# FKGSOFTWARE/TERRA-GAN

Hardware: AMD Instinct MI355X
Metric: DSM tiles/sec train-step (G+D) at 256x256 bs=16 (higher is better)
Workload: dtype f32; 1 GPU; BASELINE configs[1]: 256x256 1-ch DSM tiles, batch 16 per GPU, fp32, PConv-UNet G + PatchGAN D + L1/VGG-perceptual/TV/boundary(0.5) losses + 2x Adam; global_batch=16, tile=256, parallelism=single-gpu, launch=eager, vgg_weights=deterministic stand-in (ImageNet weights not fetchable offline; same FLOPs), vgg_trunk=forward Winograd F(2x2,3x3), dgrads F(4x4,3x3) (DESIGN 2b)

## Files before the change

terra-gan_amd/csrc/igemm_params.h:

```cpp
#pragma once
#include "common.h"

struct BnIn {
    const float *mean, *rstd, *gamma, *beta;
    int act;
    float slope;
};
struct IGemmParams {
    const float* src;
    const float* amask;
    const float* wmat;
    const float* bias;
    const float* rowscale;
    float* dst;
    float* ws;
    int B, IH, IW, C;
    int OH, OW, N, M;
    int DH, DW, ds, dy0, dx0;
    int TH, TW, ss, tstep, sy0, sx0;
    int KW, kstep, ky0, kx0;
    int Kfull, Ktot;
    int nchunks, T;
    int splits, steps_per_split;
    int act;
    float slope;
    int accumulate;
    int bf16;
    const float* gate;
    int gate_act;
    float gate_slope;
    const float* w_raw;
    long w_sn, w_sk, w_stap;
    float* wino_u;
    int wino4;
    int wino_ready;
    float* pool_dst;
    int pool_done;
    unsigned char* pool_code;
    int pool_only;
    BnIn in_bn;
    const uint32_t* gate_bits;
    int gate_bits_done;
    const TgSparseMap* sparse;
    int sparse_pix_done;
};
__device__ __forceinline__ float gate_factor(const IGemmParams& p, size_t idx) {
    const float gv = p.gate[idx];
    return gv > 0.f ? 1.f : (p.gate_act == TG_ACT_LEAKY ? p.gate_slope : 0.f);
}

int gate_bits_apply_launch(float* dx, const uint32_t* bits, int64_t rows, int C, hipStream_t s);

struct IGemmMulti {
    IGemmParams c[4];
    int zbeg[5];
};

struct WgradParams {
    const float* x;
    const float* amask;
    const float* dy;
    float* out;
    int B, H, W, C, Ho, Wo, Cout, k, stride, pad;
    int Mpix, Ktot, T, splits, steps_per_split;
    int nx, ny;
    int rowseg;
    BnIn in_bn;
};

enum SmallRoute {
    SR_NONE = 0,
    SR_C1MFMA = 100,
    SR_C1CONV = 110,
    SR_TO1CONVW = 200,
    SR_TO1_LDS = 300,
    SR_TO1_LDS_BNIN = 301,
    SR_TO1_LDS_MAP = 302,
    SR_TO1CONV64 = 400,
    SR_MULTI22_LDS = 500,
    SR_MULTI22 = 501,
    SR_C1WGRAD_MFMA = 600,
    SR_C1WGRAD_MFMA_BIAS = 610,
    SR_C1WGRAD = 620,
    SR_TO1WGRADW = 700,
    SR_TO1WGRAD_LDS = 800,
    SR_TO1WGRAD_LDS_BNIN = 801,
    SR_TO1WGRAD64 = 900,
};

enum WinoRoute {
    WR_NONE = 0,
    WR_FIRST = 1,
    WR_PIPE = WR_FIRST + 4,
    WR_QUEUED = WR_FIRST + 8,
    WR_MAP = WR_FIRST + 16,
    WR_MAP_LIST = WR_FIRST + 18,
    WR_W22_FAST = 2, WR_W22_QUEUED = 4,
    WR_WGRAD = WR_FIRST,
};

bool smallconv_fwd_applies(const IGemmParams& p);
int smallconv_fwd_launch(const IGemmParams& p, hipStream_t s, int* route = nullptr);
bool smallconv_to1_map_ok(const IGemmParams& p);
int pix_zero_launch(float* dx, const uint64_t* pix, int B, int H, int W, hipStream_t s);
bool smallconv_to1_multi_applies(const IGemmParams* cls, int ncls);
int smallconv_to1_multi_launch(const IGemmParams* cls, int ncls, hipStream_t s, int* route = nullptr);
bool smallconv_wgrad_applies(const WgradParams& p);
bool smallconv_bnin_fwd_ok(const IGemmParams& p);
bool smallconv_bnin_wgrad_ok(const WgradParams& p);
size_t smallconv_wgrad_ws_floats(const WgradParams& p);
int smallconv_wgrad_launch(const WgradParams& p, float* dw, float* ws, size_t ws_floats, hipStream_t s, float* db = nullptr,
                           int* db_done = nullptr, int* route = nullptr);
```

terra-gan_amd/csrc/wino22.inc:

```
#pragma once

struct W22Geom {
    int tiles_x, tiles_y, total_work, chunks_per_split, nt;
    int sy_min, sx_min;
    int s2d;
    int XH, XW, XC;
    int interleave;
    int* qctr;
    int ncls;
};
constexpr int W22_PTS = 9;
constexpr int W22_V = W22_PTS * 64 * 8;
constexpr int W22_PPIX = 17 * 17;
constexpr int W22_P = W22_PPIX * 8;
constexpr int W22_LDS_FLOATS = 4 * W22_V + W22_P + 8;

__device__ void wino22_weights_body(const float* __restrict__ w, float* __restrict__ U, int N, int K, const W22Weights& ww) {
    const int NT = N / WINO_BN;
    const size_t per = (size_t)N * K, total = per * ww.ncls;
    for (size_t idx0 = (size_t)blockIdx.x * 256 + threadIdx.x; idx0 < total; idx0 += (size_t)gridDim.x * 256) {
        const int cls = (int)(idx0 / per);
        const size_t idx = idx0 - cls * per;
        const int blk = (int)(idx >> 9), KC = K >> 3;
        const int k = (blk % KC) * 8 + (int)(idx & 7), n = (blk / KC) * WINO_BN + (int)((idx >> 3) & 63);
        const int ph = ww.by_phase ? k / ww.cin : cls, kc = ww.by_phase ? k - ph * ww.cin : k;
        const int dy = ph >> 1, dx = ph & 1;
        const float* wp = w + (size_t)n * ww.sn + (size_t)kc * ww.sk;
        float g[2][2];
#pragma unroll
        for (int u = 0; u < 2; ++u)
#pragma unroll
            for (int v = 0; v < 2; ++v) g[u][v] = wp[(size_t)((2 * ww.tyu[u] + dy) * 4 + (2 * ww.txv[v] + dx)) * ww.cin];
        const int row = n % WINO_BN;
        float* ub = U + cls * (per * W22_PTS) + ((size_t)(k >> 3) * NT + n / WINO_BN) * W22_V + row * 8 + wino_swz(row, k & 7);
        const float r0[3] = {g[0][0], g[0][0] + g[0][1], g[0][1]};
        const float r2[3] = {g[1][0], g[1][0] + g[1][1], g[1][1]};
#pragma unroll
        for (int b = 0; b < 3; ++b) {
            ub[(0 * 3 + b) * (WINO_BN * 8)] = r0[b];
            ub[(1 * 3 + b) * (WINO_BN * 8)] = r0[b] + r2[b];
            ub[(2 * 3 + b) * (WINO_BN * 8)] = r2[b];
        }
    }
}
__global__ __launch_bounds__(256) void wino22_weights_kernel(const float* __restrict__ w, float* __restrict__ U, int N, int K,
                                                             W22Weights ww) {
    wino22_weights_body(w, U, N, K, ww);
}

template <bool FAST, bool GATED, bool STEAL>
__global__ __launch_bounds__(WINO_THREADS) void wino22_kernel(const IGemmParams p, const W22Geom q, const float* __restrict__ U) {
    extern __shared__ __attribute__((aligned(16))) float smem[];
    float* Vs = smem;
    float* Us = smem + 2 * W22_V;
    float* Ps = smem + 4 * W22_V;

    const int tid = threadIdx.x, lane = tid & 63, wave = __builtin_amdgcn_readfirstlane(tid >> 6);
    const int mw = wave & 1, nw = (wave >> 1) & 1, xh = wave >> 2;
    __shared__ int wq_slot[2];
    WinoWork<STEAL> wk;
    wk.init(q.total_work, q.interleave, q.qctr, wq_slot);

    int n0, oy0, ox0, b, cls;
    const float* Ub;
    int s_iy[2], s_ix[2];
    int32_t poff[2];
    float pmul[2];
    int i_nt, i_tx, i_ty;
    auto locate = [&]() {
        const int item = wk.item;
        i_nt = item % q.nt;
        int tile = item / q.nt;
        cls = tile % q.ncls;
        tile /= q.ncls;
        i_tx = tile % q.tiles_x;
        tile /= q.tiles_x;
        i_ty = tile % q.tiles_y;
        b = tile / q.tiles_y;
    };
    const bool p1_ok = ((tid + WINO_THREADS) >> 1) < W22_PPIX;
    auto set_phase = [&](int ph) {
#pragma unroll
        for (int i = 0; i < 2; ++i) {
            int iy = s_iy[i], ix = s_ix[i], H = p.IH, W = p.IW, Cc = p.C;
            if (q.s2d) {
                iy = 2 * iy + (ph >> 1) - 1;
                ix = 2 * ix + (ph & 1) - 1;
                H = q.XH; W = q.XW; Cc = q.XC;
            }
            const bool ok = (i == 0 || p1_ok) && iy >= 0 && iy < H && ix >= 0 && ix < W;
            const int32_t pix = ok ? (b * H + iy) * W + ix : 0;
            poff[i] = pix * Cc + 4 * (tid & 1);
            if constexpr (FAST) poff[i] = ok ? poff[i] * 4 : (int32_t)0x80000000u;
            else pmul[i] = ok ? (p.amask ? p.amask[pix] : 1.f) : 0.f;
        }
    };
    const auto srsrc = __builtin_amdgcn_make_buffer_rsrc(
        const_cast<float*>(p.src), 0, FAST ? (int)(q.s2d ? (size_t)p.B * q.XH * q.XW * q.XC * 4 : (size_t)p.B * p.IH * p.IW * p.C * 4) : 0, 0x00020000);
    const auto ursrc = __builtin_amdgcn_make_buffer_rsrc(const_cast<float*>(U), 0, FAST ? (int)((size_t)q.ncls * W22_PTS * p.N * p.C * 4) : 0,
                                                         0x00020000);
    auto decode = [&]() {
        n0 = i_nt * WINO_BN; oy0 = i_ty * 16; ox0 = i_tx * 16;
        Ub = U + (size_t)cls * ((size_t)W22_PTS * p.N * p.C) + (size_t)i_nt * W22_V;
        const int py0 = oy0 + (q.ncls > 1 ? -(cls >> 1) : q.sy_min), px0 = ox0 + (q.ncls > 1 ? -(cls & 1) : q.sx_min);
#pragma unroll
        for (int i = 0; i < 2; ++i) {
            const int pp = (tid + WINO_THREADS * i) >> 1, spy = pp / 17, spx = pp - spy * 17;
            s_iy[i] = py0 + spy;
            s_ix[i] = px0 + spx;
        }
    };
    const int c_begin = blockIdx.z * q.chunks_per_split;
    const int c_end = min(p.C >> 3, c_begin + q.chunks_per_split);
    const int c_last = c_end - 1;
    const size_t ustep = (size_t)q.nt * W22_V;
    const int cpp = q.s2d ? (q.XC >> 3) : (p.C >> 3);
    const int ph_begin = c_begin / cpp;

    f32x4 ru[3], rp[2];
    int cur_ph, c_base, c_next;
    auto start_phase = [&](int ph) { cur_ph = ph; c_base = ph * cpp; c_next = c_base + cpp; set_phase(ph); };
    auto pload1 = [&](int c, int i) {
        if constexpr (FAST) rp[i] = __builtin_bit_cast(f32x4, __builtin_amdgcn_raw_buffer_load_b128(srsrc, poff[i], (c - c_base) * 32, 0));
        else rp[i] = *reinterpret_cast<const f32x4*>(p.src + poff[i] + (c - c_base) * 8);
    };
    const int u_idx[3] = {tid, tid + WINO_THREADS, tid < 128 ? tid + 2 * WINO_THREADS : tid};
    const size_t u_base = (size_t)W22_PTS * p.N * p.C;
    auto uload1 = [&](int c, int j) {
        if constexpr (FAST)
            ru[j] = __builtin_bit_cast(f32x4, __builtin_amdgcn_raw_buffer_load_b128(
                ursrc, 16 * u_idx[j], (int)(((size_t)cls * u_base + (size_t)i_nt * W22_V + (size_t)c * ustep) * 4), 0));
        else ru[j] = *reinterpret_cast<const f32x4*>(Ub + (size_t)c * ustep + 4 * u_idx[j]);
    };
    auto pstore1 = [&](int i) {
        f32x4 v = rp[i];
        if constexpr (!FAST) {
            v = v * pmul[i];
#pragma unroll
            for (int e = 0; e < 4; ++e) v[e] = pmul[i] != 0.f ? v[e] : 0.f;
        }
        if (i == 0 || p1_ok) *reinterpret_cast<f32x4*>(Ps + 4 * (tid + WINO_THREADS * i)) = v;
    };
    auto ustore1 = [&](int buf, int j) {
        if (j < 2 || tid < 128) *reinterpret_cast<f32x4*>(Us + buf * W22_V + 4 * (tid + WINO_THREADS * j)) = ru[j];
    };

    const int t_quad = lane & 1, t_tile = (lane >> 1) + 32 * (wave & 1), t_a = min(wave >> 1, 2);
    const bool t_on = wave < 6;
    const int t_src0 = ((2 * (t_tile >> 3) + t_a) * 17 + 2 * (t_tile & 7)) * 8 + 4 * t_quad;
    const int t_src1 = ((2 * (t_tile >> 3) + 1) * 17 + 2 * (t_tile & 7)) * 8 + 4 * t_quad;
    const int t_dst = (t_a * 3) * 512 + t_tile * 8 + (((t_quad ^ (t_tile >> 4)) & 1) << 2);
    f32x4 td[2][3], tt[3];
    auto t_read1 = [&](int k) {
        td[k / 3][k % 3] = *reinterpret_cast<const f32x4*>(Ps + ((k / 3) ? t_src1 : t_src0) + (k % 3) * 8);
    };
    auto t_row1 = [&](int j) {
        if (t_a == 1) tt[j] = td[0][j];
        else tt[j] = td[0][j] - td[1][j];
    };
    auto t_col1 = [&](int buf, int k) {
        const f32x4 v = k == 0 ? tt[0] - tt[1] : k == 1 ? tt[1] : tt[2] - tt[1];
        *reinterpret_cast<f32x4*>(Vs + buf * W22_V + t_dst + k * 512) = v;
    };

    const int pt0 = xh == 0 ? 0 : 6;
    const int arow = 32 * mw + (lane & 31), brow = 32 * nw + (lane & 31);
    const int a_off = pt0 * 512 + arow * 8 + ((((lane >> 5) ^ (arow >> 4)) & 1) << 2);
    const int b_off = pt0 * 512 + brow * 8 + ((((lane >> 5) ^ (brow >> 4)) & 1) << 2);

    if (wk.item < 0 || c_begin >= c_end) { wk.done(q.qctr); return; }
    locate();
    decode();
    start_phase(ph_begin);
#pragma unroll
    for (int i = 0; i < 2; ++i) pload1(c_begin, i);
#pragma unroll
    for (int j = 0; j < 3; ++j) uload1(c_begin, j);

    for (;;) {
        f32x16 acc[6];
#pragma unroll
        for (int i = 0; i < 6; ++i)
#pragma unroll
            for (int r = 0; r < 16; ++r) acc[i][r] = 0.f;
        {
#pragma unroll
            for (int i = 0; i < 2; ++i) pstore1(i);
#pragma unroll
            for (int j = 0; j < 3; ++j) ustore1(0, j);
            {
                const int c1 = min(c_begin + 1, c_last);
                if (c1 >= c_next) start_phase(cur_ph + 1);
#pragma unroll
                for (int i = 0; i < 2; ++i) pload1(c1, i);
#pragma unroll
                for (int j = 0; j < 3; ++j) uload1(c1, j);
            }
            wino_barrier();
            if (t_on) {
#pragma unroll
                for (int k = 0; k < 6; ++k) t_read1(k);
#pragma unroll
                for (int j = 0; j < 3; ++j) t_row1(j);
#pragma unroll
                for (int k = 0; k < 3; ++k) t_col1(0, k);
            }
            wino_barrier();
            f32x4 fa[2], fb[2];
            fa[0] = *reinterpret_cast<const f32x4*>(Vs + a_off);
            fb[0] = *reinterpret_cast<const f32x4*>(Us + b_off);
            int cur = 0;
            for (int c = c_begin; c < c_end; ++c) {
                const int nxt = cur ^ 1;
                const int c2 = min(c + 2, c_last);
                const float* Vc = Vs + cur * W22_V + a_off;
                const float* Uc = Us + cur * W22_V + b_off;
                const float* Vn = Vs + nxt * W22_V + a_off;
                const float* Un = Us + nxt * W22_V + b_off;
                wino_static_for(std::make_integer_sequence<int, 24>{}, [&](auto tc) {
                    constexpr int t = decltype(tc)::value;
                    constexpr int xi = t >> 2, e = t & 3;
                    if constexpr (t < 2) pstore1(t);
                    if constexpr (t == 2) {
                        if (c2 >= c_next) start_phase(cur_ph + 1);
                        pload1(c2, 0);
                    }
                    if constexpr (t == 3) pload1(c2, 1);
                    if constexpr (t == 4) wino_barrier();
                    if constexpr (t >= 5 && t < 8) { if (t_on) { t_read1(t - 5); t_read1(3 + t - 5); } }
                    if constexpr (t >= 8 && t < 11) { if (t_on) t_row1(t - 8); }
                    if constexpr (t >= 12 && t < 15) { if (t_on) t_col1(nxt, t - 12); }
                    if constexpr (t >= 15 && t < 18) ustore1(nxt, t - 15);
                    if constexpr (t >= 18 && t < 21) uload1(c2, t - 18);
                    if constexpr (t == 21) wino_barrier();
                    if constexpr (e == 0 && xi < 5) {
                        if (xi + 1 < 3 || xh == 0) {
                            fa[(xi + 1) & 1] = *reinterpret_cast<const f32x4*>(Vc + (xi + 1) * 512);
                            fb[(xi + 1) & 1] = *reinterpret_cast<const f32x4*>(Uc + (xi + 1) * 512);
                        }
                    }
                    if constexpr (t == 22) {
                        fa[0] = *reinterpret_cast<const f32x4*>(Vn);
                        fb[0] = *reinterpret_cast<const f32x4*>(Un);
                    }
                    __builtin_amdgcn_sched_barrier(0);
                    if (xi < 3 || xh == 0) acc[xi] = __builtin_amdgcn_mfma_f32_32x32x2f32(fa[xi & 1][e], fb[xi & 1][e], acc[xi], 0, 0, 0);
                    __builtin_amdgcn_sched_barrier(0);
                });
                cur = nxt;
            }
        }
        const int e_n0 = n0, e_oy0 = oy0, e_ox0 = ox0, e_b = b, e_cls = cls;
        const int wq_next = wk.next(wq_slot);
        const bool more_items = wq_next >= 0;
        const int wq_pulled = wk.request(wq_next);
        wino_barrier();

        float* X = smem;
        float* scratch = smem + 2 * W22_V + wave * (32 * 36);
        f32x16 own[2];
#pragma unroll
        for (int j = 0; j < 2; ++j) {
            float* xs = X + ((nw * 2 + mw) * 2 + j) * 1024 + lane;
            if (xh == 0) {
#pragma unroll
                for (int r = 0; r < 16; ++r) {
                    const float s0 = acc[j][r] + acc[j + 1][r], s1 = acc[3 + j][r] + acc[4 + j][r];
                    own[j][r] = s0 + s1;
                    xs[r * 64] = s1;
                }
            } else {
#pragma unroll
                for (int r = 0; r < 16; ++r) own[j][r] = acc[j][r] + acc[j + 1][r];
            }
        }
        if (more_items) {
            wk.item = wq_next;
            locate();
            decode();
            start_phase(ph_begin);
#pragma unroll
            for (int i = 0; i < 2; ++i) pload1(c_begin, i);
#pragma unroll
            for (int j = 0; j < 3; ++j) uload1(c_begin, j);
        }
        wino_barrier();
        const int e_dy0 = q.ncls > 1 ? 1 - (e_cls >> 1) : p.dy0, e_dx0 = q.ncls > 1 ? 1 - (e_cls & 1) : p.dx0;
        f32x4 bq = {0.f, 0.f, 0.f, 0.f};
        float rsq[2][4] = {{1.f, 1.f, 1.f, 1.f}, {1.f, 1.f, 1.f, 1.f}};
        if (p.splits == 1) {
            if (p.bias) bq = *reinterpret_cast<const f32x4*>(p.bias + e_n0 + 32 * nw + 4 * (lane & 7));
            if (p.rowscale) {
#pragma unroll
                for (int j = 0; j < 2; ++j)
#pragma unroll
                    for (int t4 = 0; t4 < 4; ++t4) {
                        const int t = 32 * mw + (lane >> 3) + 8 * t4;
                        const int oy = min(e_oy0 + 2 * (t >> 3) + xh, p.OH - 1), ox = min(e_ox0 + 2 * (t & 7) + j, p.OW - 1);
                        rsq[j][t4] = p.rowscale[((size_t)e_b * p.DH + (oy * p.ds + e_dy0)) * p.DW + (ox * p.ds + e_dx0)];
                    }
            }
        }
        f32x4 gq[GATED ? 2 : 1][GATED ? 4 : 1];
        if constexpr (GATED) {
#pragma unroll
            for (int j = 0; j < 2; ++j)
#pragma unroll
                for (int t4 = 0; t4 < 4; ++t4) {
                    const int t = 32 * mw + (lane >> 3) + 8 * t4;
                    const int oy = min(e_oy0 + 2 * (t >> 3) + xh, p.OH - 1), ox = min(e_ox0 + 2 * (t & 7) + j, p.OW - 1);
                    const size_t pix = ((size_t)e_b * p.DH + (oy * p.ds + e_dy0)) * p.DW + (ox * p.ds + e_dx0);
                    gq[j][t4] = *reinterpret_cast<const f32x4*>(p.gate + pix * p.N + e_n0 + 32 * nw + 4 * (lane & 7));
                }
        }
#pragma unroll
        for (int j = 0; j < 2; ++j) {
            f32x16 y = own[j];
            if (xh == 1) {
                const float* xr = X + ((nw * 2 + mw) * 2 + j) * 1024 + lane;
#pragma unroll
                for (int r = 0; r < 16; ++r) y[r] += xr[r * 64];
            }
            tile_rows4i(scratch, y, lane, [&](int t4, int rr, int cc, f32x4 v4) {
                const int t = 32 * mw + rr;
                const int oy = e_oy0 + 2 * (t >> 3) + xh, ox = e_ox0 + 2 * (t & 7) + j;
                const int nb = e_n0 + 32 * nw + cc;
                if (oy >= p.OH || ox >= p.OW) return;
                if (p.splits > 1) {
                    const size_t m = ((size_t)e_b * p.OH + oy) * p.OW + ox;
                    *reinterpret_cast<f32x4*>(p.ws + (((size_t)e_cls * p.splits + blockIdx.z) * p.M + m) * p.N + nb) = v4;
                } else {
                    const size_t pix = ((size_t)e_b * p.DH + (oy * p.ds + e_dy0)) * p.DW + (ox * p.ds + e_dx0);
                    *reinterpret_cast<f32x4*>(p.dst + pix * p.N + nb) = epilogue4(p, v4, pix, nb, GATED ? &gq[GATED ? j : 0][GATED ? t4 : 0] : nullptr, &rsq[j][t4], &bq);
                }
            });
        }
        wk.publish(wq_pulled, wq_slot);
        if (!more_items) break;
        wino_barrier();
        wk.advance(wq_next);
    }
    wk.done(q.qctr);
}

static bool wino22_enabled() {
    static const bool off = getenv("TG_NO_WINO") != nullptr || getenv("TG_NO_WINO22") != nullptr;
    return !off;
}
static bool wino22_fwd_geom_ok(const TgConv* g) {
    return wino22_enabled() && g->precision != TG_PREC_BF16 && g->k == 4 && g->stride == 2 && g->pad == 1 && (g->H % 2) == 0 &&
           (g->W % 2) == 0 && g->Ho == g->H / 2 && g->Wo == g->W / 2 && (g->Cin % 8) == 0 && (g->Cout % WINO_BN) == 0 && g->Ho >= 16 &&
           g->Wo >= 16;
}
static bool wino22_dgrad_geom_ok(const TgConv* g) {
    return wino22_enabled() && g->precision != TG_PREC_BF16 && g->k == 4 && g->stride == 2 && g->pad == 1 && (g->H % 2) == 0 &&
           (g->W % 2) == 0 && g->Ho == g->H / 2 && g->Wo == g->W / 2 && (g->Cout % 8) == 0 && (g->Cin % WINO_BN) == 0 && g->Ho >= 16 &&
           g->Wo >= 16;
}
static size_t wino22_u_floats(const TgConv* g) { return align_up((size_t)4 * W22_PTS * g->Cin * g->Cout, 64); }

static int launch_wino22(const TgConv* g, IGemmParams& p, int dgrad, size_t ws_floats_avail, hipStream_t s) {
    W22Geom q = {};
    W22Weights ww = {};
    p.B = g->B;
    p.OH = g->Ho; p.OW = g->Wo;
    p.M = g->B * g->Ho * g->Wo;
    ww.cin = g->Cin;
    if (!dgrad) {
        p.IH = g->Ho + 1; p.IW = g->Wo + 1; p.C = 4 * g->Cin; p.N = g->Cout;
        p.DH = g->Ho; p.DW = g->Wo; p.ds = 1; p.dy0 = 0; p.dx0 = 0;
        q.s2d = 1; q.XH = g->H; q.XW = g->W; q.XC = g->Cin; q.ncls = 1;
        q.sy_min = 0; q.sx_min = 0;
        ww.sn = 16L * g->Cin; ww.sk = 1; ww.by_phase = 1; ww.ncls = 1; ww.k_fast = 1;
        ww.tyu[0] = 0; ww.tyu[1] = 1; ww.txv[0] = 0; ww.txv[1] = 1;
    } else {
        p.IH = g->Ho; p.IW = g->Wo; p.C = g->Cout; p.N = g->Cin;
        p.DH = g->H; p.DW = g->W; p.ds = 2;
        q.s2d = 0; q.ncls = 4;
        ww.sn = 1; ww.sk = 16L * g->Cin; ww.by_phase = 0; ww.ncls = 4; ww.k_fast = 0;
        ww.tyu[0] = 1; ww.tyu[1] = 0; ww.txv[0] = 1; ww.txv[1] = 0;
    }
    q.tiles_x = cdiv(p.OW, 16);
    q.tiles_y = cdiv(p.OH, 16);
    q.nt = p.N / WINO_BN;
    q.total_work = q.tiles_x * q.tiles_y * p.B * q.nt * q.ncls;
    q.interleave = wino_interleave_ok((size_t)W22_PTS * p.N * p.C * sizeof(float));
    const int nchunks = p.C / 8;
    int splits = 1;
    if (nchunks >= 16) {
        int smax = nchunks / 8 < 16 ? nchunks / 8 : 16;
        while (smax > 1 && (size_t)smax * p.M * p.N * q.ncls > ws_floats_avail) --smax;
        splits = choose_splits(q.total_work, smax, WINO_PLAN_CUS);
    }
    q.chunks_per_split = cdiv(nchunks, splits);
    p.splits = cdiv(nchunks, q.chunks_per_split);
    p.Ktot = 4 * p.C;
    TgWprepItem it = {};
    it.kind = 3; it.N = p.N; it.K = p.C; it.w = p.w_raw; it.out = p.wino_u; it.w22 = ww;
    int rc = TG_OK;
    const auto transform = [&]() -> int {
        hipLaunchKernelGGL(wino22_weights_kernel, dim3(ew_grid((int64_t)p.N * p.C * q.ncls, 256)), dim3(256), 0, s, p.w_raw, p.wino_u, p.N,
                           p.C, ww);
        TG_CHECK_LAUNCH("wino22_weights_kernel");
        return TG_OK;
    };
    if (wino_prep(p, it, transform, &rc)) return rc;
    static const bool no_fast = getenv("TG_WINO_NO_FAST") != nullptr;
    const size_t src_bytes = (size_t)g->B * (dgrad ? (size_t)g->Ho * g->Wo * g->Cout : (size_t)g->H * g->W * g->Cin) * 4;
    const bool fast = !no_fast && p.amask == nullptr && src_bytes < ((size_t)1 << 31) && wino22_u_floats(g) * 4 < ((size_t)1 << 31);
    const bool gated = p.gate != nullptr && p.splits == 1;
    typedef void (*W22Kern)(const IGemmParams, const W22Geom, const float*);
    static const W22Kern kerns[8] = {wino22_kernel<false, false, false>, wino22_kernel<false, true, false>, wino22_kernel<true, false, false>,
                                     wino22_kernel<true, true, false>, wino22_kernel<false, false, true>, wino22_kernel<false, true, true>,
                                     wino22_kernel<true, false, true>, wino22_kernel<true, true, true>};
    static LdsOptIn opts[8];
    q.qctr = wino_queue_block(s, p.splits, q.total_work);
    const int ki = (q.qctr ? 4 : 0) + (fast ? 2 : 0) + (gated ? 1 : 0);
    const double mtot = (double)p.M * q.ncls;
    const WinoProf pf = {0, 4022, (int)mtot, 2.0 * mtot * (double)p.N * p.Ktot,
                         4.0 * ((double)g->B * (dgrad ? g->Ho * g->Wo * g->Cout : g->H * g->W * g->Cin) + 16.0 * g->Cin * g->Cout +
                                mtot * p.N + (p.rowscale ? mtot : 0.0)), WR_FIRST + ki};
    if ((rc = wino_launch(kerns[ki], opts[ki], (size_t)W22_LDS_FLOATS * sizeof(float), "wino22_kernel", p, q, pf, false, s))) return rc;
    if (p.splits > 1) {
        IGemmMulti pm = {};
        for (int c = 0; c < q.ncls; ++c) {
            pm.c[c] = p;
            pm.c[c].ws = p.ws + (size_t)c * p.splits * p.M * p.N;
            if (q.ncls > 1) { pm.c[c].dy0 = 1 - (c >> 1); pm.c[c].dx0 = 1 - (c & 1); }
        }
        hipLaunchKernelGGL(igemm_splitk_epilogue_multi, dim3(ew_grid((int64_t)p.M * p.N, 256), q.ncls), dim3(256), 0, s, pm);
        TG_CHECK_LAUNCH("igemm_splitk_epilogue_multi");
    }
    return TG_OK;
}

struct W22WgradGeom {
    int strips_x, tiles_y, nstrips, steps_per_split, splits, ntco, ntci, ctiles;
};
constexpr int W22_XR = 3 * 17 * WG_PITCH;
constexpr int W22_DR = 2 * 16 * WG_PITCH;
constexpr int W22_WG_LDS_FLOATS = 4 * W22_V + W22_XR + W22_DR;

__global__ __launch_bounds__(WINO_THREADS) void wino22_wgrad_kernel(const WgradParams p, const W22WgradGeom q, float* __restrict__ slabs) {
    extern __shared__ __attribute__((aligned(16))) float smem[];
    float* As = smem;
    float* Bs = smem + 2 * W22_V;
    float* Xr = smem + 4 * W22_V;
    float* Dr = Xr + W22_XR;

    const int tid = threadIdx.x, lane = tid & 63, wave = __builtin_amdgcn_readfirstlane(tid >> 6);
    const int mw = wave & 1, nw = (wave >> 1) & 1, xh = wave >> 2;
    const int work = xcd_remap(blockIdx.x, q.ntco * q.ntci * q.splits);
    const int tco = work % q.ntco, tci = (work / q.ntco) % q.ntci, split = work / (q.ntco * q.ntci);
    const int ph = tci / q.ctiles, ct = tci - ph * q.ctiles;
    const int pdy = (ph >> 1) - 1, pdx = (ph & 1) - 1;
    const int s_begin = split * q.steps_per_split;
    const int s_end = min(q.nstrips, s_begin + q.steps_per_split);

    const int k = lane & 7, qd = (lane >> 3) + 8 * (wave & 1), a = min(wave >> 1, 2);
    const bool t_on = wave < 6;
    int icol[4];
#pragma unroll
    for (int e = 0; e < 4; ++e) icol[e] = (3 * a) * 512 + (qd + 16 * e) * 8 + ((((k >> 2) ^ e) & 1) << 2) + (k & 3);
    const int xrd0 = (a * 17 + 2 * k) * WG_PITCH + 4 * qd, xrd1 = (17 + 2 * k) * WG_PITCH + 4 * qd;
    const int drd = (2 * k) * WG_PITCH + 4 * qd;

    const auto xrsrc = __builtin_amdgcn_make_buffer_rsrc(const_cast<float*>(p.x), 0, (int)((size_t)p.B * p.H * p.W * p.C * 4), 0x00020000);
    const auto drsrc = __builtin_amdgcn_make_buffer_rsrc(const_cast<float*>(p.dy), 0, (int)((size_t)p.B * p.Ho * p.Wo * p.Cout * 4), 0x00020000);
    const uint32_t OOB = 0xFFFFFFF0u;

    int xs_r[2], xs_px[2], xs_lds[2];
    bool xs_on[2];
#pragma unroll
    for (int i = 0; i < 2; ++i) {
        const int idx = tid + WINO_THREADS * i;
        const int ps = idx >> 4;
        xs_on[i] = ps < 3 * 17;
        xs_r[i] = ps / 17;
        xs_px[i] = ps - xs_r[i] * 17;
        xs_lds[i] = ps * WG_PITCH + 4 * (idx & 15);
    }
    const uint32_t xs_ch = (uint32_t)(ct * 64 + 4 * (tid & 15)) * 4u;
    const int ds_i = tid >> 8, ds_px = (tid >> 4) & 15, ds_lds = (tid >> 4) * WG_PITCH + 4 * (tid & 15);
    const uint32_t ds_ch = (uint32_t)(tco * 64 + 4 * (tid & 15)) * 4u;

    f32x4 rx[2][2], rd[2];
    int ls = s_begin, lsx = s_begin % q.strips_x, lty = (s_begin / q.strips_x) % q.tiles_y, lb = s_begin / (q.strips_x * q.tiles_y);
    auto raw_load = [&](auto setc) {
        constexpr int SET = decltype(setc)::value;
        const bool live = ls < s_end;
#pragma unroll
        for (int i = 0; i < 2; ++i) {
            const int py = 2 * (2 * lty + xs_r[i]) + pdy, px = 2 * (16 * lsx + xs_px[i]) + pdx;
            const bool ok = live && xs_on[i] && py >= 0 && py < p.H && px >= 0 && px < p.W;
            const uint32_t off = ok ? (((uint32_t)(lb * p.H + py) * p.W + px) * (uint32_t)p.C) * 4u + xs_ch : OOB;
            rx[SET][i] = __builtin_bit_cast(f32x4, __builtin_amdgcn_raw_buffer_load_b128(xrsrc, off, 0, 0));
        }
        {
            const int oy = 2 * lty + ds_i, ox = 16 * lsx + ds_px;
            const bool ok = live && oy < p.Ho && ox < p.Wo;
            const uint32_t off = ok ? (((uint32_t)(lb * p.Ho + oy) * p.Wo + ox) * (uint32_t)p.Cout) * 4u + ds_ch : OOB;
            rd[SET] = __builtin_bit_cast(f32x4, __builtin_amdgcn_raw_buffer_load_b128(drsrc, off, 0, 0));
        }
        ++ls;
        if (++lsx == q.strips_x) { lsx = 0; if (++lty == q.tiles_y) { lty = 0; ++lb; } }
    };
    auto raw_store = [&](auto setc) {
        constexpr int SET = decltype(setc)::value;
#pragma unroll
        for (int i = 0; i < 2; ++i)
            if (xs_on[i]) *reinterpret_cast<f32x4*>(Xr + xs_lds[i]) = rx[SET][i];
        *reinterpret_cast<f32x4*>(Dr + ds_lds) = rd[SET];
    };
    using Set0 = std::integral_constant<int, 0>;
    using Set1 = std::integral_constant<int, 1>;
    f32x4 xr[2][3], dr[2][2], tt[3], rr[2];
    auto x_read = [&](int j) {
        xr[0][j] = *reinterpret_cast<const f32x4*>(Xr + xrd0 + j * WG_PITCH);
        xr[1][j] = *reinterpret_cast<const f32x4*>(Xr + xrd1 + j * WG_PITCH);
    };
    auto d_read = [&](int i) {
        dr[i][0] = *reinterpret_cast<const f32x4*>(Dr + drd + (i * 16) * WG_PITCH);
        dr[i][1] = *reinterpret_cast<const f32x4*>(Dr + drd + (i * 16 + 1) * WG_PITCH);
    };
    auto x_rows = [&]() {
#pragma unroll
        for (int j = 0; j < 3; ++j) {
            if (a == 1) tt[j] = xr[0][j];
            else tt[j] = xr[0][j] - xr[1][j];
        }
    };
    auto d_rows = [&]() {
#pragma unroll
        for (int j = 0; j < 2; ++j) rr[j] = a == 0 ? dr[0][j] : (a == 1 ? dr[0][j] + dr[1][j] : dr[1][j]);
    };
    auto x_out = [&](int buf, int b, int h) {
        const f32x4 v = b == 0 ? tt[0] - tt[1] : b == 1 ? tt[1] : tt[2] - tt[1];
        float* dst = Bs + buf * W22_V + b * 512;
        dst[icol[2 * h]] = v[2 * h];
        dst[icol[2 * h + 1]] = v[2 * h + 1];
    };
    auto d_out = [&](int buf, int b, int h) {
        const f32x4 v = b == 0 ? rr[0] : b == 1 ? rr[0] + rr[1] : rr[1];
        float* dst = As + buf * W22_V + b * 512;
        dst[icol[2 * h]] = v[2 * h];
        dst[icol[2 * h + 1]] = v[2 * h + 1];
    };

    const int pt0 = xh == 0 ? 0 : 6;
    const int arow = 32 * mw + (lane & 31), brow = 32 * nw + (lane & 31);
    const int a_off = pt0 * 512 + arow * 8 + ((((lane >> 5) ^ (arow >> 4)) & 1) << 2);
    const int b_off = pt0 * 512 + brow * 8 + ((((lane >> 5) ^ (brow >> 4)) & 1) << 2);

    f32x16 acc[6];
#pragma unroll
    for (int i = 0; i < 6; ++i)
#pragma unroll
        for (int r = 0; r < 16; ++r) acc[i][r] = 0.f;

    if (s_begin < s_end) {
        raw_load(Set0{});
        raw_store(Set0{});
        raw_load(Set0{});
        raw_load(Set1{});
        wino_barrier();
        if (t_on) {
#pragma unroll
            for (int j = 0; j < 3; ++j) x_read(j);
            d_read(0);
            d_read(1);
            x_rows();
            d_rows();
#pragma unroll
            for (int b = 0; b < 3; ++b) { x_out(0, b, 0); x_out(0, b, 1); d_out(0, b, 0); d_out(0, b, 1); }
        }
        wino_barrier();
        f32x4 fa[2], fb[2];
        fa[0] = *reinterpret_cast<const f32x4*>(As + a_off);
        fb[0] = *reinterpret_cast<const f32x4*>(Bs + b_off);
        int cur = 0;
        auto kstep = [&](auto setc) {
            const int nxt = cur ^ 1;
            const float* Ac = As + cur * W22_V + a_off;
            const float* Bc = Bs + cur * W22_V + b_off;
            const float* An = As + nxt * W22_V + a_off;
            const float* Bn = Bs + nxt * W22_V + b_off;
            wino_static_for(std::make_integer_sequence<int, 24>{}, [&](auto tc) {
                constexpr int t = decltype(tc)::value;
                constexpr int xi = t >> 2, e = t & 3;
                if constexpr (t == 0) raw_store(setc);
                if constexpr (t == 1) raw_load(setc);
                if constexpr (t == 2) wino_barrier();
                if constexpr (t >= 3 && t < 6) { if (t_on) x_read(t - 3); }
                if constexpr (t == 6) { if (t_on) { d_read(0); d_read(1); } }
                if constexpr (t == 7) { if (t_on) x_rows(); }
                if constexpr (t >= 8 && t < 14) { if (t_on) x_out(nxt, (t - 8) >> 1, t & 1); }
                if constexpr (t == 13) { if (t_on) d_rows(); }
                if constexpr (t >= 14 && t < 20) { if (t_on) d_out(nxt, (t - 14) >> 1, t & 1); }
                if constexpr (t == 20) wino_barrier();
                if constexpr (e == 0 && xi < 5) {
                    if (xi + 1 < 3 || xh == 0) {
                        fa[(xi + 1) & 1] = *reinterpret_cast<const f32x4*>(Ac + (xi + 1) * 512);
                        fb[(xi + 1) & 1] = *reinterpret_cast<const f32x4*>(Bc + (xi + 1) * 512);
                    }
                }
                if constexpr (t == 22) {
                    fa[0] = *reinterpret_cast<const f32x4*>(An);
                    fb[0] = *reinterpret_cast<const f32x4*>(Bn);
                }
                __builtin_amdgcn_sched_barrier(0);
                if (xi < 3 || xh == 0) acc[xi] = __builtin_amdgcn_mfma_f32_32x32x2f32(fa[xi & 1][e], fb[xi & 1][e], acc[xi], 0, 0, 0);
                __builtin_amdgcn_sched_barrier(0);
            });
            cur = nxt;
        };
        for (int s = s_begin; s < s_end; s += 2) {
            kstep(Set0{});
            if (s + 1 < s_end) kstep(Set1{});
        }
    }
    float* slab = slabs + ((size_t)work * W22_PTS + pt0) * 4096;
    const int npts = xh == 0 ? 6 : 3;
#pragma unroll
    for (int i = 0; i < 6; ++i) {
        if (i < npts) {
#pragma unroll
            for (int r = 0; r < 16; ++r) {
                const int row = 32 * mw + (r & 3) + 8 * (r >> 2) + 4 * (lane >> 5);
                slab[(size_t)i * 4096 + row * 64 + 32 * nw + (lane & 31)] = acc[i][r];
            }
        }
    }
}

__global__ __launch_bounds__(256) void wino22_wgrad_reduce_kernel(const float* __restrict__ slabs, float* __restrict__ dw, int Cout,
                                                                  int Cin, int ntco, int ntci, int splits) {
    const int total = Cout * 4 * Cin;
    const int ctiles = Cin / 64;
    for (int idx = blockIdx.x * 256 + threadIdx.x; idx < total; idx += gridDim.x * 256) {
        const int col = idx & 63, row = (idx >> 6) & 63, tile = idx >> 12;
        const int tco = tile % ntco, tci = tile / ntco;
        float u[W22_PTS];
#pragma unroll
        for (int i = 0; i < W22_PTS; ++i) u[i] = 0.f;
        const size_t sstride = (size_t)ntci * ntco * W22_PTS * 4096;
        const float* sl = slabs + ((size_t)tile * W22_PTS) * 4096 + row * 64 + col;
        int sp = 0;
        for (; sp + 4 <= splits; sp += 4) {
            float v[4][W22_PTS];
#pragma unroll
            for (int k = 0; k < 4; ++k)
#pragma unroll
                for (int i = 0; i < W22_PTS; ++i) v[k][i] = sl[(size_t)(sp + k) * sstride + (size_t)i * 4096];
#pragma unroll
            for (int k = 0; k < 4; ++k)
#pragma unroll
                for (int i = 0; i < W22_PTS; ++i) u[i] += v[k][i];
        }
        for (; sp < splits; ++sp)
#pragma unroll
            for (int i = 0; i < W22_PTS; ++i) u[i] += sl[(size_t)sp * sstride + (size_t)i * 4096];
        const int ph = tci / ctiles, ct = tci - ph * ctiles;
        const int co = tco * 64 + 4 * (row & 15) + (row >> 4), c = ct * 64 + 4 * (col & 15) + (col >> 4);
        const int dy = ph >> 1, dx = ph & 1;
#pragma unroll
        for (int ty = 0; ty < 2; ++ty)
#pragma unroll
            for (int tx = 0; tx < 2; ++tx)
                dw[((size_t)(co * 4 + 2 * ty + dy) * 4 + 2 * tx + dx) * Cin + c] =
                    (u[ty * 3 + tx] + u[ty * 3 + tx + 1]) + (u[(ty + 1) * 3 + tx] + u[(ty + 1) * 3 + tx + 1]);
    }
}

static bool wino22_wgrad_ok(const TgConv* g, const float* in_mask) {
    static const bool off = getenv("TG_NO_WINO22_WGRAD") != nullptr;
    if (off || !wino22_enabled() || in_mask != nullptr || g->precision == TG_PREC_BF16) return false;
    if (g->k != 4 || g->stride != 2 || g->pad != 1 || (g->H % 2) || (g->W % 2) || g->Ho != g->H / 2 || g->Wo != g->W / 2) return false;
    if ((g->Cin % 64) != 0 || (g->Cout % 64) != 0 || g->Ho < 16 || g->Wo < 16) return false;
    if ((size_t)g->B * g->H * g->W * g->Cin * 4 >= ((size_t)1 << 31) || (size_t)g->B * g->Ho * g->Wo * g->Cout * 4 >= ((size_t)1 << 31))
        return false;
    return true;
}
static W22WgradGeom wino22_wgrad_plan(const TgConv* g) {
    W22WgradGeom q = {};
    q.strips_x = cdiv(g->Wo, 16);
    q.tiles_y = cdiv(g->Ho, 2);
    q.nstrips = g->B * q.tiles_y * q.strips_x;
    q.ntco = g->Cout / 64;
    q.ctiles = g->Cin / 64;
    q.ntci = 4 * q.ctiles;
    const int tiles = q.ntco * q.ntci;
    int smax = q.nstrips / 8 < 512 ? q.nstrips / 8 : 512;
    if (smax < 1) smax = 1;
    const int splits = choose_splits_k(tiles, smax, WINO_PLAN_CUS, q.nstrips, 0.03);
    q.steps_per_split = cdiv(q.nstrips, splits);
    q.splits = cdiv(q.nstrips, q.steps_per_split);
    return q;
}
static size_t wino22_wgrad_ws_floats(const TgConv* g) {
    if (!wino22_wgrad_ok(g, nullptr)) return 0;
    const W22WgradGeom q = wino22_wgrad_plan(g);
    return (size_t)q.splits * q.ntco * q.ntci * W22_PTS * 4096;
}
static int launch_wino22_wgrad(const TgConv* g, const WgradParams& p, float* dw, float* ws, hipStream_t s) {
    const W22WgradGeom q = wino22_wgrad_plan(g);
    const size_t lds = (size_t)W22_WG_LDS_FLOATS * sizeof(float);
    static LdsOptIn opt;
    if (int rc = lds_opt_in(opt, reinterpret_cast<const void*>(wino22_wgrad_kernel), lds, "wino22 wgrad")) return rc;
    {
        const double by = 4.0 * ((double)p.B * p.H * p.W * p.C + (double)p.Mpix * p.Cout + (double)p.Cout * p.Ktot);
        ProfScope ps(s, 1, 2.0 * p.Mpix * (double)p.Cout * p.Ktot, by, p.Cout, p.Ktot, p.Mpix, p.C, q.splits, 4122);
        ps.r.route = WR_WGRAD;
        hipLaunchKernelGGL(wino22_wgrad_kernel, dim3(q.ntco * q.ntci * q.splits), dim3(WINO_THREADS), lds, s, p, q, ws);
    }
    TG_CHECK_LAUNCH("wino22_wgrad_kernel");
    hipLaunchKernelGGL(wino22_wgrad_reduce_kernel, dim3(ew_grid((int64_t)g->Cout * 4 * g->Cin, 256)), dim3(256), 0, s, ws, dw, g->Cout,
                       g->Cin, q.ntco, q.ntci, q.splits);
    TG_CHECK_LAUNCH("wino22_wgrad_reduce_kernel");
    return TG_OK;
}
```

Before: 1077 tiles/s.

## Add wide-N Winograd F(2x2) kernel computing two output-channel tiles per block

Adds a wino22w kernel in which each work item covers 2*WINO_BN output channels, so every input-tile transform is shared across twice as many filters and the work count is halved. It is enabled by default when the fast path applies, N divides evenly, there is no split-K, and enough work remains to fill the CUs. The aim is to cut redundant input loads and transforms per FLOP. In exchange it uses more LDS and registers per block, which can lower occupancy, and leaves fewer work items for load balancing.

```diff
diff --git a/terra-gan_amd/csrc/igemm_params.h b/terra-gan_amd/csrc/igemm_params.h
--- a/terra-gan_amd/csrc/igemm_params.h
+++ b/terra-gan_amd/csrc/igemm_params.h
@@ -96,6 +96,7 @@
     WR_MAP = WR_FIRST + 16,
     WR_MAP_LIST = WR_FIRST + 18,
     WR_W22_FAST = 2, WR_W22_QUEUED = 4,
+    WR_W22_WIDE = 8,
     WR_WGRAD = WR_FIRST,
 };
 
diff --git a/terra-gan_amd/csrc/wino22.inc b/terra-gan_amd/csrc/wino22.inc
--- a/terra-gan_amd/csrc/wino22.inc
+++ b/terra-gan_amd/csrc/wino22.inc
@@ -343,9 +343,267 @@
     wk.done(q.qctr);
 }
 
+constexpr int W22W_U = 2 * W22_V;
+constexpr int W22W_LDS_FLOATS = 2 * W22_V + 2 * W22W_U + W22_P + 8;
+
+template <bool GATED, bool STEAL>
+__global__ __launch_bounds__(WINO_THREADS) void wino22w_kernel(const IGemmParams p, const W22Geom q, const float* __restrict__ U) {
+    extern __shared__ __attribute__((aligned(16))) float smem[];
+    float* Vs = smem;
+    float* Us = smem + 2 * W22_V;
+    float* Ps = smem + 2 * W22_V + 2 * W22W_U;
+
+    const int tid = threadIdx.x, lane = tid & 63, wave = __builtin_amdgcn_readfirstlane(tid >> 6);
+    const int mw = wave & 1, nw = wave >> 1;
+    __shared__ int wq_slot[2];
+    WinoWork<STEAL> wk;
+    wk.init(q.total_work, q.interleave, q.qctr, wq_slot);
+
+    int n0, oy0, ox0, b, cls;
+    int py0, px0;
+    int32_t poff[2];
+    int i_nt, i_tx, i_ty;
+    auto locate = [&]() {
+        const int item = wk.item;
+        i_nt = item % q.nt;
+        int tile = item / q.nt;
+        cls = tile % q.ncls;
+        tile /= q.ncls;
+        i_tx = tile % q.tiles_x;
+        tile /= q.tiles_x;
+        i_ty = tile % q.tiles_y;
+        b = tile / q.tiles_y;
+    };
+    const bool p1_ok = ((tid + WINO_THREADS) >> 1) < W22_PPIX;
+    auto set_phase = [&](int ph) {
+        int st = tid;
+        asm volatile("" : "+v"(st));
+#pragma unroll
+        for (int i = 0; i < 2; ++i) {
+            const int pp = (st + WINO_THREADS * i) >> 1, spy = pp / 17, spx = pp - spy * 17;
+            int iy = py0 + spy, ix = px0 + spx, H = p.IH, W = p.IW, Cc = p.C;
+            if (q.s2d) {
+                iy = 2 * iy + (ph >> 1) - 1;
+                ix = 2 * ix + (ph & 1) - 1;
+                H = q.XH; W = q.XW; Cc = q.XC;
+            }
+            const bool ok = (i == 0 || p1_ok) && iy >= 0 && iy < H && ix >= 0 && ix < W;
+            const int32_t pix = ok ? (b * H + iy) * W + ix : 0;
+            poff[i] = ok ? (pix * Cc + 4 * (st & 1)) * 4 : (int32_t)0x80000000u;
+        }
+    };
+    const auto srsrc = __builtin_amdgcn_make_buffer_rsrc(
+        const_cast<float*>(p.src), 0, (int)(q.s2d ? (size_t)p.B * q.XH * q.XW * q.XC * 4 : (size_t)p.B * p.IH * p.IW * p.C * 4), 0x00020000);
+    const auto ursrc = __builtin_amdgcn_make_buffer_rsrc(const_cast<float*>(U), 0, (int)((size_t)q.ncls * W22_PTS * p.N * p.C * 4), 0x00020000);
+    auto decode = [&]() {
+        n0 = i_nt * (2 * WINO_BN); oy0 = i_ty * 16; ox0 = i_tx * 16;
+        py0 = oy0 + (q.ncls > 1 ? -(cls >> 1) : q.sy_min);
+        px0 = ox0 + (q.ncls > 1 ? -(cls & 1) : q.sx_min);
+    };
+    const int c_begin = 0, c_end = p.C >> 3, c_last = c_end - 1;
+    const size_t ustep = (size_t)(p.N / WINO_BN) * W22_V;
+    const int cpp = q.s2d ? (q.XC >> 3) : (p.C >> 3);
+
+    f32x4 ru[5], rp[2];
+    int cur_ph, c_base, c_next;
+    auto start_phase = [&](int ph) { cur_ph = ph; c_base = ph * cpp; c_next = c_base + cpp; set_phase(ph); };
+    auto pload1 = [&](int c, int i) {
+        rp[i] = __builtin_bit_cast(f32x4, __builtin_amdgcn_raw_buffer_load_b128(srsrc, poff[i], (c - c_base) * 32, 0));
+    };
+    const size_t u_base = (size_t)W22_PTS * p.N * p.C;
+    const int u_last = tid < 256 ? tid + 4 * WINO_THREADS : tid;
+    auto uload1 = [&](int c, int j) {
+        ru[j] = __builtin_bit_cast(f32x4, __builtin_amdgcn_raw_buffer_load_b128(
+            ursrc, 16 * (j < 4 ? tid + WINO_THREADS * j : u_last), (int)(((size_t)cls * u_base + (size_t)i_nt * W22W_U + (size_t)c * ustep) * 4), 0));
+    };
+    auto pstore1 = [&](int i) {
+        if (i == 0 || p1_ok) *reinterpret_cast<f32x4*>(Ps + 4 * (tid + WINO_THREADS * i)) = rp[i];
+    };
+    auto ustore1 = [&](int buf, int j) {
+        if (j < 4 || tid < 256) *reinterpret_cast<f32x4*>(Us + buf * W22W_U + 4 * (tid + WINO_THREADS * j)) = ru[j];
+    };
+
+    const int t_quad = lane & 1, t_tile = (lane >> 1) + 32 * (wave & 1), t_a = min(wave >> 1, 2);
+    const bool t_on = wave < 6;
+    const int t_src0 = ((2 * (t_tile >> 3) + t_a) * 17 + 2 * (t_tile & 7)) * 8 + 4 * t_quad;
+    const int t_src1 = ((2 * (t_tile >> 3) + 1) * 17 + 2 * (t_tile & 7)) * 8 + 4 * t_quad;
+    const int t_dst = (t_a * 3) * 512 + t_tile * 8 + (((t_quad ^ (t_tile >> 4)) & 1) << 2);
+    f32x4 tp[2], tm;
+    auto t_read1 = [&](int j) {
+        tp[0] = *reinterpret_cast<const f32x4*>(Ps + t_src0 + j * 8);
+        tp[1] = *reinterpret_cast<const f32x4*>(Ps + t_src1 + j * 8);
+    };
+    auto t_row1 = [&]() -> f32x4 { return t_a == 1 ? tp[0] : tp[0] - tp[1]; };
+    auto t_col1 = [&](int buf, int k, f32x4 v) {
+        if (t_on) *reinterpret_cast<f32x4*>(Vs + buf * W22_V + t_dst + k * 512) = v;
+    };
+
+    const int arow = 32 * mw + (lane & 31), brow = 32 * (nw & 1) + (lane & 31);
+    const int a_off = arow * 8 + ((((lane >> 5) ^ (arow >> 4)) & 1) << 2);
+    const int b_off = (nw >> 1) * W22_V + brow * 8 + ((((lane >> 5) ^ (brow >> 4)) & 1) << 2);
+
+    if (wk.item < 0 || c_begin >= c_end) { wk.done(q.qctr); return; }
+    locate();
+    decode();
+    start_phase(0);
+#pragma unroll
+    for (int i = 0; i < 2; ++i) pload1(c_begin, i);
+#pragma unroll
+    for (int j = 0; j < 5; ++j) uload1(c_begin, j);
+
+    for (;;) {
+        f32x16 acc[W22_PTS];
+#pragma unroll
+        for (int i = 0; i < W22_PTS; ++i)
+#pragma unroll
+            for (int r = 0; r < 16; ++r) acc[i][r] = 0.f;
+        {
+#pragma unroll
+            for (int i = 0; i < 2; ++i) pstore1(i);
+#pragma unroll
+            for (int j = 0; j < 5; ++j) ustore1(0, j);
+            {
+                const int c1 = min(c_begin + 1, c_last);
+                if (c1 >= c_next) start_phase(cur_ph + 1);
+#pragma unroll
+                for (int i = 0; i < 2; ++i) pload1(c1, i);
+#pragma unroll
+                for (int j = 0; j < 5; ++j) uload1(c1, j);
+            }
+            wino_barrier();
+            t_read1(1);
+            tm = t_row1();
+            t_col1(0, 1, tm);
+            t_read1(0);
+            t_col1(0, 0, t_row1() - tm);
+            t_read1(2);
+            t_col1(0, 2, t_row1() - tm);
+            wino_barrier();
+            f32x4 fa[2], fb[2];
+            fa[0] = *reinterpret_cast<const f32x4*>(Vs + a_off);
+            fb[0] = *reinterpret_cast<const f32x4*>(Us + b_off);
+            int cur = 0;
+            for (int c = c_begin; c < c_end; ++c) {
+                const int nxt = cur ^ 1;
+                const int c2 = min(c + 2, c_last);
+                const float* Vc = Vs + cur * W22_V + a_off;
+                const float* Uc = Us + cur * W22W_U + b_off;
+                const float* Vn = Vs + nxt * W22_V + a_off;
+                const float* Un = Us + nxt * W22W_U + b_off;
+                wino_static_for(std::make_integer_sequence<int, 36>{}, [&](auto tc) {
+                    constexpr int t = decltype(tc)::value;
+                    constexpr int xi = t >> 2, e = t & 3;
+                    if constexpr (t < 2) pstore1(t);
+                    if constexpr (t == 2) {
+                        if (c2 >= c_next) start_phase(cur_ph + 1);
+                        pload1(c2, 0);
+                    }
+                    if constexpr (t == 3) pload1(c2, 1);
+                    if constexpr (t == 4) wino_barrier();
+                    if constexpr (t == 5) t_read1(1);
+                    if constexpr (t == 8) { tm = t_row1(); t_col1(nxt, 1, tm); t_read1(0); }
+                    if constexpr (t == 11) { t_col1(nxt, 0, t_row1() - tm); t_read1(2); }
+                    if constexpr (t == 14) t_col1(nxt, 2, t_row1() - tm);
+                    if constexpr (t >= 17 && t < 22) ustore1(nxt, t - 17);
+                    if constexpr (t >= 23 && t < 28) uload1(c2, t - 23);
+                    if constexpr (t == 32) wino_barrier();
+                    if constexpr (e == 0 && xi < 8) {
+                        fa[(xi + 1) & 1] = *reinterpret_cast<const f32x4*>(Vc + (xi + 1) * 512);
+                        fb[(xi + 1) & 1] = *reinterpret_cast<const f32x4*>(Uc + (xi + 1) * 512);
+                    }
+                    if constexpr (t == 33) {
+                        fa[1] = *reinterpret_cast<const f32x4*>(Vn);
+                        fb[1] = *reinterpret_cast<const f32x4*>(Un);
+                    }
+                    __builtin_amdgcn_sched_barrier(0);
+                    acc[xi] = __builtin_amdgcn_mfma_f32_32x32x2f32(fa[xi & 1][e], fb[xi & 1][e], acc[xi], 0, 0, 0);
+                    __builtin_amdgcn_sched_barrier(0);
+                });
+                fa[0] = fa[1];
+                fb[0] = fb[1];
+                cur = nxt;
+            }
+        }
+        const int e_n0 = n0, e_oy0 = oy0, e_ox0 = ox0, e_b = b, e_cls = cls;
+        const int wq_next = wk.next(wq_slot);
+        const bool more_items = wq_next >= 0;
+        const int wq_pulled = wk.request(wq_next);
+        wino_barrier();
+
+        int el = lane;
+        asm volatile("" : "+v"(el));
+        float* scratch = smem + 2 * W22_V + wave * (32 * 36);
+        f32x16 rs[3][2];
+#pragma unroll
+        for (int a = 0; a < 3; ++a)
+#pragma unroll
+            for (int j = 0; j < 2; ++j)
+#pragma unroll
+                for (int r = 0; r < 16; ++r) rs[a][j][r] = acc[3 * a + j][r] + acc[3 * a + j + 1][r];
+        const int e_dy0 = q.ncls > 1 ? 1 - (e_cls >> 1) : p.dy0, e_dx0 = q.ncls > 1 ? 1 - (e_cls & 1) : p.dx0;
+        f32x4 bq = {0.f, 0.f, 0.f, 0.f};
+        if (p.bias) bq = *reinterpret_cast<const f32x4*>(p.bias + e_n0 + 32 * nw + 4 * (el & 7));
+#pragma unroll
+        for (int xh = 0; xh < 2; ++xh) {
+            if (xh == 1 && more_items) {
+                wk.item = wq_next;
+                locate();
+                decode();
+                start_phase(0);
+#pragma unroll
+                for (int i = 0; i < 2; ++i) pload1(c_begin, i);
+#pragma unroll
+                for (int j = 0; j < 5; ++j) uload1(c_begin, j);
+            }
+#pragma unroll
+            for (int j = 0; j < 2; ++j) {
+                float rsq[4] = {1.f, 1.f, 1.f, 1.f};
+                if (p.rowscale) {
+#pragma unroll
+                    for (int t4 = 0; t4 < 4; ++t4) {
+                        const int t = 32 * mw + (el >> 3) + 8 * t4;
+                        const int oy = min(e_oy0 + 2 * (t >> 3) + xh, p.OH - 1), ox = min(e_ox0 + 2 * (t & 7) + j, p.OW - 1);
+                        rsq[t4] = p.rowscale[((size_t)e_b * p.DH + (oy * p.ds + e_dy0)) * p.DW + (ox * p.ds + e_dx0)];
+                    }
+                }
+                f32x4 gq[GATED ? 4 : 1];
+                if constexpr (GATED) {
+#pragma unroll
+                    for (int t4 = 0; t4 < 4; ++t4) {
+                        const int t = 32 * mw + (el >> 3) + 8 * t4;
+                        const int oy = min(e_oy0 + 2 * (t >> 3) + xh, p.OH - 1), ox = min(e_ox0 + 2 * (t & 7) + j, p.OW - 1);
+                        const size_t pix = ((size_t)e_b * p.DH + (oy * p.ds + e_dy0)) * p.DW + (ox * p.ds + e_dx0);
+                        gq[t4] = *reinterpret_cast<const f32x4*>(p.gate + pix * p.N + e_n0 + 32 * nw + 4 * (el & 7));
+                    }
+                }
+                f32x16 y;
+#pragma unroll
+                for (int r = 0; r < 16; ++r) y[r] = rs[xh][j][r] + rs[xh + 1][j][r];
+                tile_rows4i(scratch, y, el, [&](int t4, int rr, int cc, f32x4 v4) {
+                    const int t = 32 * mw + rr;
+                    const int oy = e_oy0 + 2 * (t >> 3) + xh, ox = e_ox0 + 2 * (t & 7) + j;
+                    const int nb = e_n0 + 32 * nw + cc;
+                    if (oy >= p.OH || ox >= p.OW) return;
+                    const size_t pix = ((size_t)e_b * p.DH + (oy * p.ds + e_dy0)) * p.DW + (ox * p.ds + e_dx0);
+                    *reinterpret_cast<f32x4*>(p.dst + pix * p.N + nb) = epilogue4(p, v4, pix, nb, GATED ? &gq[GATED ? t4 : 0] : nullptr, &rsq[t4], &bq);
+                });
+            }
+        }
+        wk.publish(wq_pulled, wq_slot);
+        if (!more_items) break;
+        wino_barrier();
+        wk.advance(wq_next);
+    }
+    wk.done(q.qctr);
+}
+
 static bool wino22_enabled() {
     static const bool off = getenv("TG_NO_WINO") != nullptr || getenv("TG_NO_WINO22") != nullptr;
     return !off;
+}
+static bool wino22_wide_enabled() {
+    const char* e = getenv("TG_WINO22_WIDE");
+    return e == nullptr || atoi(e) != 0;
 }
 static bool wino22_fwd_geom_ok(const TgConv* g) {
     return wino22_enabled() && g->precision != TG_PREC_BF16 && g->k == 4 && g->stride == 2 && g->pad == 1 && (g->H % 2) == 0 &&
@@ -414,12 +672,21 @@
                                      wino22_kernel<true, true, false>, wino22_kernel<false, false, true>, wino22_kernel<false, true, true>,
                                      wino22_kernel<true, false, true>, wino22_kernel<true, true, true>};
     static LdsOptIn opts[8];
+    const bool wide = wino22_wide_enabled() && fast && (p.N % (2 * WINO_BN)) == 0 && p.splits == 1 && q.total_work / 2 >= WINO_PLAN_CUS;
+    if (wide) { q.nt /= 2; q.total_work /= 2; }
+    static const W22Kern kernsw[4] = {wino22w_kernel<false, false>, wino22w_kernel<true, false>, wino22w_kernel<false, true>,
+                                      wino22w_kernel<true, true>};
+    static LdsOptIn optsw[4];
     q.qctr = wino_queue_block(s, p.splits, q.total_work);
     const int ki = (q.qctr ? 4 : 0) + (fast ? 2 : 0) + (gated ? 1 : 0);
     const double mtot = (double)p.M * q.ncls;
     const WinoProf pf = {0, 4022, (int)mtot, 2.0 * mtot * (double)p.N * p.Ktot,
                          4.0 * ((double)g->B * (dgrad ? g->Ho * g->Wo * g->Cout : g->H * g->W * g->Cin) + 16.0 * g->Cin * g->Cout +
-                                mtot * p.N + (p.rowscale ? mtot : 0.0)), WR_FIRST + ki};
+                                mtot * p.N + (p.rowscale ? mtot : 0.0)), WR_FIRST + (wide ? WR_W22_WIDE : 0) + ki};
+    if (wide) {
+        const int kw = (q.qctr ? 2 : 0) + (gated ? 1 : 0);
+        return wino_launch(kernsw[kw], optsw[kw], (size_t)W22W_LDS_FLOATS * sizeof(float), "wino22w_kernel", p, q, pf, false, s);
+    }
     if ((rc = wino_launch(kerns[ki], opts[ki], (size_t)W22_LDS_FLOATS * sizeof(float), "wino22_kernel", p, q, pf, false, s))) return rc;
     if (p.splits > 1) {
         IGemmMulti pm = {};
```

Result: faster. 1091 tiles/s (median of 6 runs) (+1.2%).
